# pirz/hyperspace-1

Measured on AMD Instinct MI355X. Metric: queries/sec + index-build GB/s, TPC-H SF100 filter+join at 1/2/4/8 MI355X, higher is better.
Workload: dtype fp64

## Files before the change

### csrc/kernels/scan_filter.hip

```cpp
#include "hs_vec.h"

#define SF_BLOCK 256
#define SF_ITEMS 8
#define SF_TILE (SF_BLOCK * SF_ITEMS)
#define SF_GRID 2048
#define FIN_BLOCK 256

struct ScanParams {
  ColDesc cols[HS_MAX_COLS];
  Pred preds[HS_MAX_PREDS];
  AggSpec aggs[HS_MAX_AGGS];
  int32_t npreds;
  int32_t naggs;
  int32_t group_col;
  int32_t num_groups;
  int64_t group_base;
};

#define RANGE_WAVES 4

__device__ __forceinline__ bool range_less(const ColDesc& c, int64_t r, uint64_t key, int mode) {
  if (!col_valid(c, r)) return true;
  if (mode == 2) return false;
  const uint64_t v = hs_sortable(c, r);
// ... 47 lines not shown
  range_one(key, bucket_off, buckets, i, has_lo, lo_key, lo_incl, has_hi, hi_key, hi_incl, rstart,
            rlen, rbucket);
}

__global__ __launch_bounds__(64 * RANGE_WAVES) void hs_probe_ranges_kernel(
    ColDesc key, const int64_t* __restrict__ bucket_off, const int32_t* __restrict__ pbucket,
    const uint64_t* __restrict__ pkey, int np, int64_t* __restrict__ rstart,
    int64_t* __restrict__ rlen, int32_t* __restrict__ rbucket) {
  const int i = blockIdx.x * RANGE_WAVES + (threadIdx.x >> 6);
  if (i >= np) return;
  range_one(key, bucket_off, pbucket, i, 1, pkey[i], 1, 1, pkey[i], 1, rstart, rlen, rbucket);
}

__global__ __launch_bounds__(64 * RANGE_WAVES) void hs_range_search_dev_kernel(
    ColDesc key, const int64_t* __restrict__ bucket_off, const int32_t* __restrict__ buckets,
    int nb, const int64_t* __restrict__ bp, int64_t* __restrict__ rstart,
    int64_t* __restrict__ rlen, int32_t* __restrict__ rbucket) {
  const int i = blockIdx.x * RANGE_WAVES + (threadIdx.x >> 6);
  if (i >= nb) return;
  range_one(key, bucket_off, buckets, i, (int)bp[0], (uint64_t)bp[1], (int)bp[2], (int)bp[3],
            (uint64_t)bp[4], (int)bp[5], rstart, rlen, rbucket);
}

__global__ __launch_bounds__(64) void hs_ranges_to_tiles_kernel(const int64_t* __restrict__ rlen,
                                                                int R, int tile_rows,
                                                                int64_t* __restrict__ tile_prefix,
                                                                const int64_t* __restrict__ rstart,
                                                                int64_t align) {
  const int lane = threadIdx.x & 63;
  int64_t carry = 0;
  for (int base = 0; base < R; base += 64) {
    const int i = base + lane;
    const int64_t len = i < R ? rlen[i] + (rstart != nullptr ? (rstart[i] & (align - 1)) : 0) : 0;
    const int64_t t = (len + tile_rows - 1) / tile_rows;
    int64_t x = t;
#pragma unroll
    for (int off = 1; off < 64; off <<= 1) {
      const int64_t y = __shfl_up(x, off, 64);
      if (lane >= off) x += y;
    }
    if (i < R) tile_prefix[i] = carry + x - t;
    carry += __shfl(x, 63, 64);
  }
  if (lane == 0) tile_prefix[R] = carry;
}

// ... 40 lines not shown
  int64_t t0, t1;
  block_tile_chunk(tile_prefix[R], t0, t1);
  if (t0 < t1) {
    TileWalker tw{tile_prefix, rstart, rlen, R, 0};
    tw.init(t0);
    for (int64_t t = t0; t < t1; ++t) {
      int64_t row0, rows;
      tw.at(t, row0, rows);
      int64_t r[SF_ITEMS];
      bool act[SF_ITEMS], pass[SF_ITEMS];
      tile_rows(row0, rows, r, act);
      veval_cnf(p.preds, 0, p.npreds, p.cols, HS_MAX_COLS, r, r, act, pass);
      int g[SF_ITEMS];
#pragma unroll
      for (int i = 0; i < SF_ITEMS; ++i) g[i] = 0;
      if (GROUPED)
        vgroup(p.cols, p.group_col, HS_MAX_COLS, p.group_base, p.num_groups, r, r, pass, g);
      vaccumulate<GROUPED, SF_ITEMS>(acc, p.aggs, A, p.cols, HS_MAX_COLS, r, r, pass, g, gl);
    }
  }
  acc_flush<GROUPED, SF_BLOCK>(acc, p.aggs, A, GA, gl, psum, pcnt, pmin, pmax);
}

__global__ __launch_bounds__(FIN_BLOCK) void hs_agg_final_kernel(
    const double* __restrict__ psum, const int64_t* __restrict__ pcnt,
    const double* __restrict__ pmin, const double* __restrict__ pmax, int nblk, int GA,
    double* __restrict__ osum, int64_t* __restrict__ ocnt, double* __restrict__ omin,
    double* __restrict__ omax) {
  __shared__ double rs[FIN_BLOCK / 64], rmn[FIN_BLOCK / 64], rmx[FIN_BLOCK / 64];
  __shared__ int64_t rc[FIN_BLOCK / 64];
  const int i = blockIdx.x;
  double s = 0.0, mn = __builtin_inf(), mx = -__builtin_inf();
  int64_t c = 0;
#pragma unroll 4
  for (int b = threadIdx.x; b < nblk; b += FIN_BLOCK) {
    const int64_t o = (int64_t)b * GA + i;
    s += psum[o];
    c += pcnt[o];
    mn = fmin(mn, pmin[o]);
    mx = fmax(mx, pmax[o]);
  }
  s = hs_wave_sum(s);
  c = hs_wave_sum(c);
  mn = hs_wave_min(mn);
  mx = hs_wave_max(mx);
  const int w = threadIdx.x >> 6;
  if ((threadIdx.x & 63) == 0) {
    rs[w] = s;
    rc[w] = c;
    rmn[w] = mn;
    rmx[w] = mx;
  }
  __syncthreads();
  if (threadIdx.x == 0) {
    double ts = 0.0, tmn = __builtin_inf(), tmx = -__builtin_inf();
    int64_t tc = 0;
    for (int k = 0; k < FIN_BLOCK / 64; ++k) {
      ts += rs[k];
      tc += rc[k];
      tmn = fmin(tmn, rmn[k]);
      tmx = fmax(tmx, rmx[k]);
    }
    osum[i] = ts;
    ocnt[i] = tc;
    omin[i] = tmn;
    omax[i] = tmx;
  }
}

__global__ __launch_bounds__(SF_BLOCK) void hs_scan_count_kernel(
    ScanParams p, const int64_t* __restrict__ rstart, const int64_t* __restrict__ rlen, int R,
    const int64_t* __restrict__ tile_prefix, int64_t* __restrict__ tile_counts) {
  __shared__ int64_t red[SF_BLOCK / 64];
  int64_t t0, t1;
  block_tile_chunk(tile_prefix[R], t0, t1);
  if (t0 >= t1) return;
  TileWalker tw{tile_prefix, rstart, rlen, R, 0};
  tw.init(t0);
  for (int64_t t = t0; t < t1; ++t) {
    int64_t row0, rows;
    tw.at(t, row0, rows);
    int64_t r[SF_ITEMS];
    bool act[SF_ITEMS], pass[SF_ITEMS];
    tile_rows(row0, rows, r, act);
    veval_cnf(p.preds, 0, p.npreds, p.cols, HS_MAX_COLS, r, r, act, pass);
    int64_t cnt = 0;
#pragma unroll
    for (int i = 0; i < SF_ITEMS; ++i) cnt += pass[i] ? 1 : 0;
    cnt = hs_wave_sum(cnt);
// ... 117 lines not shown
int hs_ranges_to_tiles(const int64_t* rlen, int R, int tile_rows, int64_t* tile_prefix,
                       void* stream) {
  hipLaunchKernelGGL(hs_ranges_to_tiles_kernel, dim3(1), dim3(64), 0, (hipStream_t)stream, rlen,
                     R, tile_rows, tile_prefix, (const int64_t*)nullptr, (int64_t)1);
  return (int)hipGetLastError();
}

int hs_ranges_to_tiles_aligned(const int64_t* rstart, const int64_t* rlen, int R, int tile_rows,
                               int64_t align, int64_t* tile_prefix, void* stream) {
  hipLaunchKernelGGL(hs_ranges_to_tiles_kernel, dim3(1), dim3(64), 0, (hipStream_t)stream, rlen,
                     R, tile_rows, tile_prefix, rstart, align);
  return (int)hipGetLastError();
}

int hs_agg_final(const double* psum, const int64_t* pcnt, const double* pmin, const double* pmax,
                 int nblk, int GA, double* osum, int64_t* ocnt, double* omin, double* omax,
                 void* stream) {
  if (GA <= 0) return 0;
  hipLaunchKernelGGL(hs_agg_final_kernel, dim3(GA), dim3(FIN_BLOCK), 0, (hipStream_t)stream, psum,
                     pcnt, pmin, pmax, nblk, GA, osum, ocnt, omin, omax);
  return (int)hipGetLastError();
}

int hs_scan_agg(const ScanParams* p, const int64_t* rstart, const int64_t* rlen, int R,
                const int64_t* tile_prefix, int grid, double* psum, int64_t* pcnt, double* pmin,
                double* pmax, double* osum, int64_t* ocnt, double* omin, double* omax,
                void* stream) {
  hipStream_t s = (hipStream_t)stream;
  const bool grouped = p->group_col >= 0;
  const int GA = grouped ? p->num_groups * p->naggs : p->naggs;
  if (GA <= 0) return 0;
  if (grouped) {
    const size_t lds = (size_t)GA * 32;
    if (lds > 120 * 1024) return -5;
    hipLaunchKernelGGL(hs_scan_agg_kernel<true>, dim3(grid), dim3(SF_BLOCK), lds, s, *p, rstart,
                       rlen, R, tile_prefix, psum, pcnt, pmin, pmax);
  } else {
    hipLaunchKernelGGL(hs_scan_agg_kernel<false>, dim3(grid), dim3(SF_BLOCK), 0, s, *p, rstart,
                       rlen, R, tile_prefix, psum, pcnt, pmin, pmax);
  }
  return hs_agg_final(psum, pcnt, pmin, pmax, grid, GA, osum, ocnt, omin, omax, stream);
}

int hs_scan_count(const ScanParams* p, const int64_t* rstart, const int64_t* rlen, int R,
                  const int64_t* tile_prefix, int grid, int64_t* tile_counts, void* stream) {
  hipLaunchKernelGGL(hs_scan_count_kernel, dim3(grid), dim3(SF_BLOCK), 0, (hipStream_t)stream, *p,
// ... 23 lines not shown
```

### csrc/runtime/hs_graph.cpp

```cpp
#include <hip/hip_runtime.h>

#include <algorithm>
#include <cstdint>
#include <cstring>
#include <string>
#include <vector>

namespace {

thread_local std::string g_err;

struct HsGraph {
  hipGraph_t graph = nullptr;
  hipGraphExec_t exec = nullptr;
  hipEvent_t join = nullptr;
  std::vector<hipGraphNode_t> nodes;
  std::vector<hipKernelNodeParams> params;
};

int fail(const char* what, hipError_t e) {
  g_err = std::string(what) + ": " + hipGetErrorString(e);
  return (int)e;
}

bool sort_by_depth(std::vector<hipGraphNode_t>& all) {
  const size_t n = all.size();
  std::vector<std::vector<size_t>> deps(n);
  for (size_t k = 0; k < n; ++k) {
    size_t nd = 0;
    if (hipGraphNodeGetDependencies(all[k], nullptr, &nd) != hipSuccess) return false;
    std::vector<hipGraphNode_t> d(nd);
    if (nd && hipGraphNodeGetDependencies(all[k], d.data(), &nd) != hipSuccess) return false;
    for (size_t j = 0; j < nd; ++j) {
      size_t at = 0;
      while (at < n && all[at] != d[j]) ++at;
      if (at == n) return false;
// ... 27 lines not shown
  all.swap(out);
  return true;
}

}

extern "C" {

const char* hs_graph_last_error() { return g_err.c_str(); }

int hs_graph_capture_begin(void* stream) {
  const hipError_t e = hipStreamBeginCapture((hipStream_t)stream, hipStreamCaptureModeThreadLocal);
  return e == hipSuccess ? 0 : fail("hipStreamBeginCapture", e);
}

void* hs_graph_capture_end(void* stream, void** funcs, int nfuncs) {
  hipGraph_t graph = nullptr;
  hipError_t e = hipStreamEndCapture((hipStream_t)stream, &graph);
  if (e != hipSuccess || graph == nullptr) {
    fail("hipStreamEndCapture", e);
    return nullptr;
  }
  auto* g = new HsGraph();
  g->graph = graph;
  size_t n = 0;
  e = hipGraphGetNodes(graph, nullptr, &n);
  std::vector<hipGraphNode_t> all(n);
  if (e == hipSuccess && n) e = hipGraphGetNodes(graph, all.data(), &n);
  if (e != hipSuccess) {
    fail("hipGraphGetNodes", e);
    hipGraphDestroy(graph);
    delete g;
    return nullptr;
  }
  all.resize(n);
  if (!sort_by_depth(all)) {
    g_err = "hs_graph_capture_end: could not order the captured nodes by dependency";
    hipGraphDestroy(graph);
    delete g;
    return nullptr;
  }
  std::vector<char> taken(n, 0);
  for (int i = 0; i < nfuncs; ++i) {
    bool found = false;
    for (size_t k = 0; k < n && !found; ++k) {
      if (taken[k]) continue;
      hipGraphNodeType t;
      if (hipGraphNodeGetType(all[k], &t) != hipSuccess || t != hipGraphNodeTypeKernel) continue;
      hipKernelNodeParams p;
      std::memset(&p, 0, sizeof(p));
      if (hipGraphKernelNodeGetParams(all[k], &p) != hipSuccess) continue;
      if (p.func != funcs[i]) continue;
      taken[k] = 1;
      g->nodes.push_back(all[k]);
      g->params.push_back(p);
      found = true;
    }
    if (!found) {
      g_err = "hs_graph_capture_end: kernel node of function " + std::to_string(i) + " not found";
      hipGraphDestroy(graph);
      delete g;
      return nullptr;
    }
  }
  e = hipGraphInstantiate(&g->exec, graph, nullptr, nullptr, 0);
  if (e != hipSuccess) {
    fail("hipGraphInstantiate", e);
    hipGraphDestroy(graph);
    delete g;
    return nullptr;
  }
  return g;
}

int hs_graph_set_args(void* handle, int i, void* args, size_t size) {
  auto* g = (HsGraph*)handle;
  if (i < 0 || (size_t)i >= g->nodes.size()) {
    g_err = "hs_graph_set_args: bad node index";
    return -1;
  }
  (void)size;
  hipKernelNodeParams p = g->params[i];
  void* kp[1] = {args};
  p.kernelParams = kp;
  p.extra = nullptr;
  const hipError_t e = hipGraphExecKernelNodeSetParams(g->exec, g->nodes[i], &p);
  return e == hipSuccess ? 0 : fail("hipGraphExecKernelNodeSetParams", e);
}

int hs_graph_launch(void* handle, void* stream) {
  auto* g = (HsGraph*)handle;
  const hipError_t e = hipGraphLaunch(g->exec, (hipStream_t)stream);
  return e == hipSuccess ? 0 : fail("hipGraphLaunch", e);
}

// ... 49 lines not shown
}

int hs_event_query(void* ev) {
  const hipError_t e = hipEventQuery((hipEvent_t)ev);
  if (e == hipSuccess) return 0;
  if (e == hipErrorNotReady) return 1;
  return -fail("hipEventQuery", e);
}

int hs_event_sync(void* ev) {
  const hipError_t e = hipEventSynchronize((hipEvent_t)ev);
  return e == hipSuccess ? 0 : fail("hipEventSynchronize", e);
}

void hs_event_destroy(void* ev) {
  if (ev != nullptr) hipEventDestroy((hipEvent_t)ev);
}

void hs_graph_destroy(void* handle) {
  auto* g = (HsGraph*)handle;
  if (g == nullptr) return;
  if (g->join) hipEventDestroy(g->join);
  if (g->exec) hipGraphExecDestroy(g->exec);
  if (g->graph) hipGraphDestroy(g->graph);
  delete g;
}

}
```

### hyperspace_amd/exec/graphs.py

```python
from __future__ import annotations

import ctypes as C
import struct
import threading
from collections import OrderedDict
from typing import Optional, Tuple

import numpy as np

from ..ops import _lib as NL
from . import jit

PARAM_HEAD = 64


class _Pinned:

    def __init__(self, nbytes: int):
        self.nbytes = nbytes
        self.ptr = jit.runtime().hs_host_alloc(nbytes)
        if not self.ptr:
            raise MemoryError(f"hipHostMalloc({nbytes}) failed")

    def view(self) -> np.ndarray:
        v = getattr(self, "_view", None)
        if v is None:
            v = self._view = np.ctypeslib.as_array((C.c_uint8 * self.nbytes).from_address(self.ptr))
        return v

    def __del__(self):
        if getattr(self, "ptr", None):
            jit.runtime().hs_host_free(self.ptr)
            self.ptr = None


class _Slot:

    def __init__(self, params_bytes: int, out_bytes: int):
        self.h_params = _Pinned(max(params_bytes, 8))
        self.h_out = _Pinned(out_bytes)
        self.graph = None
        self.event = jit.runtime().hs_event_create()
        if not self.event:
            raise RuntimeError(f"hs_event_create: {jit.runtime().hs_graph_last_error().decode()}")
        self.launched = False
        self.current = None

    def done(self) -> bool:
        rc = jit.runtime().hs_event_query(self.event)
        _rt_check(rc if rc < 0 else 0, "hs_event_query")
        return rc == 0

    def wait(self) -> None:
        _rt_check(jit.runtime().hs_event_sync(self.event), "hs_event_sync")

    def __del__(self):
        R = jit.runtime()
        if getattr(self, "graph", None):
            R.hs_graph_destroy(self.graph)
            self.graph = None
        if getattr(self, "event", None):
            R.hs_event_destroy(self.event)
            self.event = None


class _Launch:

    __slots__ = ("slot", "value")

    def __init__(self, slot: _Slot):
        self.slot = slot
        self.value = None


def _rt_check(rc: int, what: str) -> None:
    if rc != 0:
        raise RuntimeError(f"{what}: {jit.runtime().hs_graph_last_error().decode()}")


class _RingGraph:
    RING = 4

    def _init_ring(self, params_bytes: int) -> None:
        self.slots = [_Slot(params_bytes, self.out[0].hs_buf.numel()) for _ in range(self.RING)]
        self._next = 0
        self._warm = False
        self.replays = 0
        self.on_side = False
        self.side_stream = None

    @property
    def graph(self):
        return self.slots[0].graph

    def _capture(self, slot: _Slot, blocks, cur) -> None:
        slot.graph = self._capture_of(lambda st: self._enqueue(slot, st, blocks), self.kernels,
                                      cur)

    def _capture_of(self, enqueue, kernels, cur):
        import torch
        R = jit.runtime()
        side = torch.cuda.Stream()
        side.wait_stream(cur)
        _rt_check(R.hs_graph_capture_begin(side.cuda_stream), "hs_graph_capture_begin")
        try:
            enqueue(side.cuda_stream)
        finally:
            fns = [k.function() for k in kernels]
            arr = (C.c_void_p * len(fns))(*fns)
            h = R.hs_graph_capture_end(side.cuda_stream, arr, len(fns))
        if not h:
            raise RuntimeError(f"graph capture: {R.hs_graph_last_error().decode()}")
        cur.wait_stream(side)
        return h

    def _take_slot(self) -> _Slot:
        slot = self.slots[self._next]
        self._next = (self._next + 1) % len(self.slots)
        prev = slot.current
        if prev is not None and prev.value is None:
            prev.value = self._read(slot)
        elif slot.launched and not slot.done():
            slot.wait()
        return slot

    def busy(self) -> bool:
        slot = self.slots[self._next - 1]
        return slot.launched and not slot.done()

    def _launch_slot(self, fill, blocks, stream=None, after=None) -> _Launch:
        import torch
        slot = self._take_slot()
        fill(slot.h_params)
        R = jit.runtime()
        if slot.graph is not None:
            st = stream.cuda_stream if stream is not None else NL.raw_stream()
            ptrs = (C.c_void_p * len(blocks))(*[C.addressof(b) for b in blocks])
            _rt_check(R.hs_graph_replay(slot.graph, len(blocks), ptrs, st,
                                        after.cuda_stream if after is not None else None,
                                        slot.event), "hs_graph_replay")
            self.replays += 1
        else:
            cur = stream if stream is not None else torch.cuda.current_stream()
            st = cur.cuda_stream
            if after is not None:
                cur.wait_stream(after)
            if not self._warm:
                self._enqueue(slot, st, blocks)
                self._warm = True
            else:
                self._capture(slot, blocks, cur)
                _rt_check(R.hs_graph_launch(slot.graph, st), "hs_graph_launch")
                self.replays += 1
            _rt_check(R.hs_event_record(slot.event, st), "hs_event_record")
        slot.launched = True
        h = _Launch(slot)
        slot.current = h
        return h

    def result(self, h: _Launch):
        if h.value is None:
            h.value = self._read(h.slot)
        return h.value

    def _read(self, slot: _Slot):
        slot.wait()
        h = slot.h_out.view()
        n = 8 * self.GA
        return (h[0:n].view(np.float64).copy(), h[n:2 * n].view(np.int64).copy(),
                h[2 * n:3 * n].view(np.float64).copy(), h[3 * n:4 * n].view(np.float64).copy())

    def _final_and_d2h(self, slot: _Slot, stream: int, grid: int, parts=None) -> None:
        L = jit.runtime()
        K = NL.lib()
        p = self.parts if parts is None else parts
        o = self.out
        NL.check(K.hs_agg_final(NL.ptr(p[0]), NL.ptr(p[1]), NL.ptr(p[2]), NL.ptr(p[3]),
                                grid, self.GA, NL.ptr(o[0]), NL.ptr(o[1]), NL.ptr(o[2]),
                                NL.ptr(o[3]), stream), "hs_agg_final")
        NL.check(L.hs_memcpy_async(slot.h_out.ptr, o[0].hs_buf.data_ptr(), slot.h_out.nbytes, 2,
                                   stream), "result D2H")


def _cbuf(block) -> "C.Array":
    b = bytes(block)
    return C.create_string_buffer(b, len(b))


class ScanAggGraph(_RingGraph):
    def __init__(self, kernel: jit.Kernel, kd: NL.ColDesc, bucket_off, nb: int, grid: int,
                 GA: int, shmem: int, device, vec: int = 0):
        import torch
        from ..ops import kernels as K
        self.kernel = kernel
        self.kernels = (kernel,)
        self.kd = kd
        self.bucket_off = bucket_off
        self.nb, self.grid, self.GA, self.shmem = nb, grid, GA, shmem
        self.vec = vec
        self.tile = jit.BLOCK * (vec or jit.SCAN_ITEMS)
        self.d_params = torch.empty(PARAM_HEAD, dtype=torch.uint8, device=device)
        self.rstart = torch.empty(nb, dtype=torch.int64, device=device)
        self.rlen = torch.empty(nb, dtype=torch.int64, device=device)
        self.rbk = torch.empty(nb, dtype=torch.int32, device=device)
        self.tp = torch.empty(nb + 1, dtype=torch.int64, device=device)
        self.parts = jit._partials(grid, GA, device)
        self.out = K.agg_outputs(GA, device)
        self._init_ring(PARAM_HEAD)

    def _enqueue(self, slot: _Slot, stream: int, blocks) -> None:
        L = jit.runtime()
        K = NL.lib()
        NL.check(L.hs_memcpy_async(self.d_params.data_ptr(), slot.h_params.ptr,
                                   slot.h_params.nbytes, 1, stream), "param H2D")
        NL.check(K.hs_range_search_dev(C.byref(self.kd), NL.ptr(self.bucket_off), None, self.nb,
                                       self.d_params.data_ptr(), NL.ptr(self.rstart),
                                       NL.ptr(self.rlen), NL.ptr(self.rbk), stream),
                 "hs_range_search_dev")
        if self.vec:
            NL.check(K.hs_ranges_to_tiles_aligned(NL.ptr(self.rstart), NL.ptr(self.rlen), self.nb,
                                                  self.tile, self.vec, NL.ptr(self.tp), stream),
                     "hs_ranges_to_tiles_aligned")
        else:
            NL.check(K.hs_ranges_to_tiles(NL.ptr(self.rlen), self.nb, self.tile,
                                          NL.ptr(self.tp), stream), "hs_ranges_to_tiles")
        self.kernel.launch_packed(self.grid, blocks[0], stream, self.shmem)
        self._final_and_d2h(slot, stream, self.grid)

    def buffers(self) -> list:
        return [self.d_params, self.rstart, self.rlen, self.rbk, self.tp, self.bucket_off,
                *self.parts, self.out[0].hs_buf]

    def values_template(self) -> dict:
        return {"rstart": self.rstart.data_ptr(), "rlen": self.rlen.data_ptr(),
                "tile_prefix": self.tp.data_ptr(), "R": self.nb,
                "psum": self.parts[0].data_ptr(), "pcnt": self.parts[1].data_ptr(),
                "pmin": self.parts[2].data_ptr(), "pmax": self.parts[3].data_ptr()}

    def launch(self, bounds: Tuple[int, int, int, int, int, int], args_block, stream=None,
               after=None) -> _Launch:
        head = struct.pack("<6q", *bounds)

        def fill(hp):
            C.memmove(hp.ptr, head, 48)
        if not isinstance(args_block, C.Array):
            args_block = _cbuf(args_block)
        return self._launch_slot(fill, (args_block,), stream, after)

    def run(self, bounds: Tuple[int, int, int, int, int, int], args_block):
        return self.result(self.launch(bounds, args_block))


def _nofill(hp) -> None:
    pass


class TwoPhaseGraph(_RingGraph):

    def __init__(self, kt: jit.Kernel, ks: jit.Kernel, grid_t: int, grid_s: int, GA: int,
                 shmem: int, device):
        from ..ops import kernels as K
        self.kt, self.ks = kt, ks
        self.kernels = (kt, ks)
        self.grid_t, self.grid_s, self.GA, self.shmem = grid_t, grid_s, GA, shmem
        self.parts = jit._partials(grid_s, GA, device)
        self.parts_b = jit._partials(grid_s, GA, device)
        self.out = K.agg_outputs(GA, device)
        self._init_ring(0)
        self.pairs: dict = {}
        self._pair_warm = False
        self.pair_replays = 0

    def _enqueue(self, slot: _Slot, stream: int, blocks) -> None:
        self.kt.launch_packed(self.grid_t, blocks[0], stream, 0)
        self.ks.launch_packed(self.grid_s, blocks[1], stream, self.shmem)
        self._final_and_d2h(slot, stream, self.grid_s)

    def _enqueue_pair(self, ktp: jit.Kernel, sa: _Slot, sb: _Slot, stream: int, blocks,
                      ksp: Optional[jit.Kernel] = None) -> None:
        ktp.launch_packed(self.grid_t, blocks[0], stream, 0)
        if ksp is not None:
            ksp.launch_packed(self.grid_s, blocks[1], stream, self.shmem)
            self._final_and_d2h(sa, stream, self.grid_s)
            self._final_and_d2h(sb, stream, self.grid_s, self.parts_b)
            return
        for slot, blk in ((sa, blocks[1]), (sb, blocks[2])):
            self.ks.launch_packed(self.grid_s, blk, stream, self.shmem)
            self._final_and_d2h(slot, stream, self.grid_s)

    def launch_pair(self, ktp: jit.Kernel, block_tp, block_sa, block_sb, single,
                    ksp: Optional[jit.Kernel] = None) -> tuple:
        import torch
        ia = self._next
        sa, sb = self._take_slot(), self._take_slot()
        blocks = (block_tp, block_sa, block_sb) if ksp is None else (block_tp, block_sa)
        R = jit.runtime()
        h = self.pairs.get(ia)
        if h is not None:
            st = NL.raw_stream()
            ptrs = (C.c_void_p * len(blocks))(*[C.addressof(b) for b in blocks])
            _rt_check(R.hs_graph_replay(h, len(blocks), ptrs, st, None, sa.event),
                      "hs_graph_replay")
            self.pair_replays += 1
        else:
            cur = torch.cuda.current_stream()
            st = cur.cuda_stream
            if not self._pair_warm:
                self._enqueue_pair(ktp, sa, sb, st, blocks, ksp)
                self._pair_warm = True
            else:
                h = self.pairs[ia] = self._capture_of(
                    lambda s_: self._enqueue_pair(ktp, sa, sb, s_, blocks, ksp),
                    (ktp, self.ks, self.ks) if ksp is None else (ktp, ksp), cur)
                _rt_check(R.hs_graph_launch(h, st), "hs_graph_launch")
                self.pair_replays += 1
            _rt_check(R.hs_event_record(sa.event, st), "hs_event_record")
        _rt_check(R.hs_event_record(sb.event, st), "hs_event_record")
        out = []
        for slot in (sa, sb):
            slot.launched = True
            slot.current = _Launch(slot)
            out.append(slot.current)
        if self._warm and (sa.graph is None or sb.graph is None):
            self._capture(sa if sa.graph is None else sb, single, torch.cuda.current_stream())
        return tuple(out)

    def __del__(self):
        pairs = getattr(self, "pairs", None)
        while pairs:
            jit.runtime().hs_graph_destroy(pairs.popitem()[1])

    def buffers(self) -> list:
        return [*self.parts, *self.parts_b, self.out[0].hs_buf]

    def partial_ptrs(self, sfx: str = "", parts=None) -> dict:
        p = self.parts if parts is None else parts
        return {"psum" + sfx: p[0].data_ptr(), "pcnt" + sfx: p[1].data_ptr(),
                "pmin" + sfx: p[2].data_ptr(), "pmax" + sfx: p[3].data_ptr()}

    def launch(self, block_t, block_s) -> _Launch:
        return self._launch_slot(_nofill, (block_t, block_s))


class GraphPending:
    __slots__ = ("graph", "handle")

    def __init__(self, graph, handle):
        self.graph, self.handle = graph, handle

    def result(self):
        return self.graph.result(self.handle)

    def done(self) -> bool:
        h = self.handle
        return h.value is not None or h.slot.current is not h or h.slot.done()


class GraphCache:

    def __init__(self, capacity: int = 64):
        self.capacity = capacity
        self._lru: "OrderedDict[tuple, ScanAggGraph]" = OrderedDict()
        self._lock = threading.Lock()

# ... 34 lines not shown
```

### hyperspace_amd/exec/jit.py

```python
from __future__ import annotations

import ctypes as C
import os
import re
import struct
import threading
from typing import Dict, List, Optional, Tuple

from ..ops import _lib as NL

ARCH = os.environ.get("HS_OFFLOAD_ARCH", "gfx950")
_HERE = os.path.dirname(os.path.dirname(os.path.abspath(__file__)))
RUNTIME_PATH = os.path.join(_HERE, "_native", "libhs_runtime.so")
CACHE_DIR = os.environ.get("HS_JIT_CACHE", os.path.join(_HERE, "_native", "jitcache"))

BLOCK = 256
from . import kernel_config as _KC
_CFG = _KC.active()
SCAN_ITEMS, SCAN_GRID, SCAN_VEC = _CFG.scan_items, _CFG.scan_grid, _CFG.scan_vec
SCAN_COMPACT, SCAN_EAGER = _CFG.scan_compact, _CFG.scan_eager
JOIN_ITEMS, JOIN_BLOCK, JOIN_LDS_KEYS, JOIN_GRID = (_CFG.join_items, _CFG.join_block,
                                                    _CFG.join_lds_keys, _CFG.join_grid)
JOIN_EAGER, JOIN_STAGE_RIGHT, JOIN_PIPELINE = (_CFG.join_eager, _CFG.join_stage_right,
                                               _CFG.join_pipeline)
# ... 40 lines not shown
                L.hs_jit_launch.restype = C.c_int
                L.hs_jit_launch.argtypes = [C.c_void_p, C.c_uint, C.c_uint, C.c_uint, C.c_void_p,
                                            C.c_void_p, C.c_size_t]
                L.hs_jit_compile_to_cache.restype = C.c_int
                L.hs_jit_compile_to_cache.argtypes = [C.c_char_p] * 4
                L.hs_jit_last_error.restype = C.c_char_p
                L.hs_host_alloc.restype = C.c_void_p
                L.hs_host_alloc.argtypes = [C.c_size_t]
                L.hs_host_free.restype = None
                L.hs_host_free.argtypes = [C.c_void_p]
                L.hs_memcpy_async.restype = C.c_int
                L.hs_memcpy_async.argtypes = [C.c_void_p, C.c_void_p, C.c_size_t, C.c_int,
                                              C.c_void_p]
                L.hs_stream_sync.restype = C.c_int
                L.hs_stream_sync.argtypes = [C.c_void_p]
                L.hs_graph_capture_begin.restype = C.c_int
                L.hs_graph_capture_begin.argtypes = [C.c_void_p]
                L.hs_graph_capture_end.restype = C.c_void_p
                L.hs_graph_capture_end.argtypes = [C.c_void_p, C.POINTER(C.c_void_p), C.c_int]
                L.hs_graph_set_args.restype = C.c_int
                L.hs_graph_set_args.argtypes = [C.c_void_p, C.c_int, C.c_void_p, C.c_size_t]
                L.hs_graph_launch.restype = C.c_int
                L.hs_graph_launch.argtypes = [C.c_void_p, C.c_void_p]
                L.hs_graph_destroy.restype = None
                L.hs_graph_destroy.argtypes = [C.c_void_p]
                L.hs_graph_replay.restype = C.c_int
                L.hs_graph_replay.argtypes = [C.c_void_p, C.c_int, C.c_void_p, C.c_void_p,
                                              C.c_void_p, C.c_void_p]
                L.hs_event_create.restype = C.c_void_p
                L.hs_event_create.argtypes = []
                L.hs_event_record.restype = C.c_int
                L.hs_event_record.argtypes = [C.c_void_p, C.c_void_p]
                L.hs_event_query.restype = C.c_int
                L.hs_event_query.argtypes = [C.c_void_p]
                L.hs_event_sync.restype = C.c_int
                L.hs_event_sync.argtypes = [C.c_void_p]
                L.hs_event_destroy.restype = None
                L.hs_event_destroy.argtypes = [C.c_void_p]
                L.hs_graph_last_error.restype = C.c_char_p
                _rt = L
    return _rt


class Args:

    def __init__(self):
# ... 1804 lines not shown
```

### hyperspace_amd/ops/_lib.py

```python
from __future__ import annotations

import ctypes as C
import os

_HERE = os.path.dirname(os.path.dirname(os.path.abspath(__file__)))
LIB_PATH = os.path.join(_HERE, "_native", "libhs_kernels.so")

MAX_COLS = 16
MAX_PREDS = 16
MAX_AGGS = 8
MAX_TERMS = 3
HASH_MAX_COLS = 8
GATHER_MAX_COLS = 32

I8, I16, I32, I64, F32, F64, BOOL, U32, U64 = range(9)
STR = 100
STRDICT = 101
PK_INT_LIT, PK_FLT_LIT, PK_INT_COL, PK_FLT_COL, PK_IS_NULL, PK_NOT_NULL, PK_IN_SET, PK_BITMAP, \
    PK_TRUE = range(9)
OP_EQ, OP_NE, OP_LT, OP_LE, OP_GT, OP_GE = range(6)
AK_SUM, AK_COUNT, AK_MIN, AK_MAX, AK_COUNT_STAR = range(5)


class ColDesc(C.Structure):
# ... 65 lines not shown


XCH_MAX_COLS = 32
XCH_MAX_DEST = 64


class XchParams(C.Structure):
    _fields_ = [("src", C.c_void_p * XCH_MAX_COLS), ("elem_bytes", C.c_int32 * XCH_MAX_COLS),
                ("ncols", C.c_int32), ("world", C.c_int32)]


class XchCopy(C.Structure):
    _fields_ = [("src", C.c_void_p), ("dst", C.c_void_p), ("count", C.c_int64),
                ("elem_bytes", C.c_int32), ("pad", C.c_int32)]


WIN_MAX_KEYS = 8
WA_SUM_I64, WA_SUM_F64, WA_COUNT, WA_MIN_I64, WA_MAX_I64, WA_MIN_F64, WA_MAX_F64 = range(7)


class WinKeys(C.Structure):
    _fields_ = [("part", ColDesc * WIN_MAX_KEYS), ("order", ColDesc * WIN_MAX_KEYS),
                ("npart", C.c_int32), ("norder", C.c_int32)]


_lib = None


class NativeMissing(RuntimeError):
    pass


def _sig(fn, restype, *args):
    fn.restype = restype
    fn.argtypes = list(args)


def bind_hip_runtime() -> None:
    import torch


def lib():
    global _lib
    if _lib is not None:
        return _lib
    if not os.path.exists(LIB_PATH):
        raise NativeMissing(f"{LIB_PATH} not built; run `python -m hyperspace_amd._native.build`")
    bind_hip_runtime()
    L = C.CDLL(LIB_PATH)
    P, I, I64, U64 = C.c_void_p, C.c_int, C.c_int64, C.c_uint64
    for name, st in (("hs_hash_params_size", HashParams), ("hs_scan_params_size", ScanParams),
                     ("hs_join_params_size", JoinParams), ("hs_sort_key_spec_size", SortKeySpec),
                     ("hs_gather_params_size", GatherParams), ("hs_xch_params_size", XchParams),
                     ("hs_xch_copy_size", XchCopy), ("hs_merge_keys_size", MergeKeys),
                     ("hs_win_keys_size", WinKeys)):
        f = getattr(L, name)
        f.restype = C.c_int
        if f() != C.sizeof(st):
            raise RuntimeError(f"ABI mismatch for {st.__name__}: lib {f()} vs ctypes {C.sizeof(st)}")
    _sig(L.hs_murmur3_bucket, I, P, I64, P, P, P)
    _sig(L.hs_murmur3_hash, I, P, I64, P, P)
    _sig(L.hs_sort_workspace_bytes, I64, I64)
    _sig(L.hs_sort_columns, I, P, I, I64, P, I, P, I64, P)
    _sig(L.hs_merge_make_keys, I, P, I64, P, P)
    _sig(L.hs_merge_round, I, P, P, P, P, P, I, I64, P)
    _sig(L.hs_scan_tmp_elems, I64, I64)
    _sig(L.hs_exclusive_scan_i64, I, P, P, I64, P, I64, P)
    _sig(L.hs_exclusive_scan_u32, I, P, P, I64, P, I64, P)
    _sig(L.hs_gather, I, P, P, I64, P)
    _sig(L.hs_gather_packed, I, P, I, I, I64, P, P, I64, P)
    _sig(L.hs_bucket_offsets, I, P, I64, I, P, P)
    _sig(L.hs_scan_tile_rows, I)
    _sig(L.hs_scan_grid, I)
    _sig(L.hs_join_tile_rows, I)
    _sig(L.hs_range_search, I, P, P, P, I, I, U64, I, I, U64, I, P, P, P, P)
    _sig(L.hs_range_search_dev, I, P, P, P, I, P, P, P, P, P)
    _sig(L.hs_ranges_to_tiles, I, P, I, I, P, P)
    _sig(L.hs_ranges_to_tiles_aligned, I, P, P, I, I, I64, P, P)
    _sig(L.hs_scan_agg, I, P, P, P, I, P, I, P, P, P, P, P, P, P, P, P)
    _sig(L.hs_scan_count, I, P, P, P, I, P, I, P, P)
    _sig(L.hs_scan_select, I, P, P, P, I, P, P, I, P, P)
    _sig(L.hs_scan_bitmap, I, P, P, P, I, P, I, I, I64, I64, P, P)
    _sig(L.hs_join_agg, I, P, P, P, P, P, I, P, I64, P, I, P, P, P, P, P, P, P, P, P)
    _sig(L.hs_agg_final, I, P, P, P, P, I, I, P, P, P, P, P)
    _sig(L.hs_join_count, I, P, P, P, P, P, I, P, I64, P, I, P, P)
    _sig(L.hs_join_emit, I, P, I, P, P, I, P, P, P, P)
    _sig(L.hs_join_spans, I, P, P, P, P, P, I, P, I64, P, I, P)
    _sig(L.hs_join_spans_sampled, I, P, P, P, P, P, P, I, I64, P, I, P, I64, P, I, I, P)
    _sig(L.hs_join_sample_stride, I)
    _sig(L.hs_join_index, I, P, I, P, P, I, P, P)
    _sig(L.hs_pq_decode_values, I, P, P, I64, I64, I64, I, P, P)
    _sig(L.hs_pq_decode_levels, I, P, P, I64, P, P)
    _sig(L.hs_pq_pack, I, P, P, I, I64, I, P, P, P)
    _sig(L.hs_pq_dict_mark, I, P, P, I, I64, I, P, P)
    _sig(L.hs_pq_dict_remap, I, P, P, I, I64, I, P, P, P)
    _sig(L.hs_pq_warmup, I, P)
    _sig(L.hs_pq_decode_pages, I, P, P, P, I, P, P)
    _sig(L.hs_pq_page_struct_size, I)
    _sig(L.hs_pq_dict_codes, I, P, I64, I, P, I, P, P, P)
    _sig(L.hs_histogram, I, P, I64, I, P, P)
    _sig(L.hs_xch_tile_rows, I)
    _sig(L.hs_xch_pack, I, P, P, I64, P, P, P, P)
    _sig(L.hs_xch_unpack, I, P, I, I64, P)
    _sig(L.hs_probe_ranges, I, P, P, P, P, I, P, P, P, P)
    _sig(L.hs_compact_result_size, I)
    _sig(L.hs_compact_probe, I, P, P, I64, I, I, P, P, P)
    _sig(L.hs_compact_probe_ws_elems, I64)
# ... 87 lines not shown
```

Baseline: 4840.

## Fold aggregate finalisation with host write into kernel and clone captured graphs

Replaces the separate agg-final kernel plus D2H memcpy with a fold kernel that writes results straight into pinned host memory, using a system fence. Range-search parameters now travel by value in kernel arguments instead of through an H2D param copy. Graphs are captured once as a prototype and cloned for the other ring slots instead of being recaptured per slot. This removes memcpy graph nodes and repeated capture cost, at the price of system-scope device writes and graphs that share ownership.

```diff
diff --git a/csrc/kernels/scan_filter.hip b/csrc/kernels/scan_filter.hip
--- a/csrc/kernels/scan_filter.hip
+++ b/csrc/kernels/scan_filter.hip
@@ -93,6 +93,25 @@
             (uint64_t)bp[4], (int)bp[5], rstart, rlen, rbucket);
 }
 
+struct RangeValArgs {
+  ColDesc key;
+  const int64_t* bucket_off;
+  const int32_t* buckets;
+  int64_t* rstart;
+  int64_t* rlen;
+  int32_t* rbucket;
+  int64_t bp[6];
+  int32_t nb;
+  int32_t pad;
+};
+
+__global__ __launch_bounds__(64 * RANGE_WAVES) void hs_range_search_val_kernel(RangeValArgs a) {
+  const int i = blockIdx.x * RANGE_WAVES + (threadIdx.x >> 6);
+  if (i >= a.nb) return;
+  range_one(a.key, a.bucket_off, a.buckets, i, (int)a.bp[0], (uint64_t)a.bp[1], (int)a.bp[2],
+            (int)a.bp[3], (uint64_t)a.bp[4], (int)a.bp[5], a.rstart, a.rlen, a.rbucket);
+}
+
 __global__ __launch_bounds__(64) void hs_ranges_to_tiles_kernel(const int64_t* __restrict__ rlen,
                                                                 int R, int tile_rows,
                                                                 int64_t* __restrict__ tile_prefix,
@@ -179,14 +198,12 @@
   acc_flush<GROUPED, SF_BLOCK>(acc, p.aggs, A, GA, gl, psum, pcnt, pmin, pmax);
 }
 
-__global__ __launch_bounds__(FIN_BLOCK) void hs_agg_final_kernel(
+__device__ __forceinline__ bool agg_final_slot(
     const double* __restrict__ psum, const int64_t* __restrict__ pcnt,
-    const double* __restrict__ pmin, const double* __restrict__ pmax, int nblk, int GA,
-    double* __restrict__ osum, int64_t* __restrict__ ocnt, double* __restrict__ omin,
-    double* __restrict__ omax) {
+    const double* __restrict__ pmin, const double* __restrict__ pmax, int nblk, int GA, int i,
+    double& ts, int64_t& tc, double& tmn, double& tmx) {
   __shared__ double rs[FIN_BLOCK / 64], rmn[FIN_BLOCK / 64], rmx[FIN_BLOCK / 64];
   __shared__ int64_t rc[FIN_BLOCK / 64];
-  const int i = blockIdx.x;
   double s = 0.0, mn = __builtin_inf(), mx = -__builtin_inf();
   int64_t c = 0;
 #pragma unroll 4
@@ -209,19 +226,70 @@
     rmx[w] = mx;
   }
   __syncthreads();
-  if (threadIdx.x == 0) {
-    double ts = 0.0, tmn = __builtin_inf(), tmx = -__builtin_inf();
-    int64_t tc = 0;
-    for (int k = 0; k < FIN_BLOCK / 64; ++k) {
-      ts += rs[k];
-      tc += rc[k];
-      tmn = fmin(tmn, rmn[k]);
-      tmx = fmax(tmx, rmx[k]);
-    }
+  if (threadIdx.x != 0) return false;
+  ts = 0.0, tmn = __builtin_inf(), tmx = -__builtin_inf();
+  tc = 0;
+  for (int k = 0; k < FIN_BLOCK / 64; ++k) {
+    ts += rs[k];
+    tc += rc[k];
+    tmn = fmin(tmn, rmn[k]);
+    tmx = fmax(tmx, rmx[k]);
+  }
+  return true;
+}
+
+__global__ __launch_bounds__(FIN_BLOCK) void hs_agg_final_kernel(
+    const double* __restrict__ psum, const int64_t* __restrict__ pcnt,
+    const double* __restrict__ pmin, const double* __restrict__ pmax, int nblk, int GA,
+    double* __restrict__ osum, int64_t* __restrict__ ocnt, double* __restrict__ omin,
+    double* __restrict__ omax) {
+  const int i = blockIdx.x;
+  double ts, tmn, tmx;
+  int64_t tc;
+  if (agg_final_slot(psum, pcnt, pmin, pmax, nblk, GA, i, ts, tc, tmn, tmx)) {
     osum[i] = ts;
     ocnt[i] = tc;
     omin[i] = tmn;
     omax[i] = tmx;
+  }
+}
+
+struct AggFoldSet {
+  const double* psum;
+  const int64_t* pcnt;
+  const double* pmin;
+  const double* pmax;
+  unsigned char* dout;
+  unsigned char* hout;
+  int32_t nblk;
+  int32_t pad;
+};
+
+struct AggFoldArgs {
+  int32_t GA;
+  int32_t nsets;
+  AggFoldSet set[2];
+};
+
+__device__ __forceinline__ void agg_fold_store(unsigned char* __restrict__ out, int GA, int i,
+                                               double ts, int64_t tc, double tmn, double tmx) {
+  const size_t n = (size_t)8 * GA;
+  ((double*)out)[i] = ts;
+  ((int64_t*)(out + n))[i] = tc;
+  ((double*)(out + 2 * n))[i] = tmn;
+  ((double*)(out + 3 * n))[i] = tmx;
+}
+
+__global__ __launch_bounds__(FIN_BLOCK) void hs_agg_fold_kernel(AggFoldArgs a) {
+  const int k = blockIdx.x / a.GA, i = blockIdx.x - k * a.GA;
+  if (k >= a.nsets) return;
+  const AggFoldSet st = k == 0 ? a.set[0] : a.set[1];
+  double ts, tmn, tmx;
+  int64_t tc;
+  if (agg_final_slot(st.psum, st.pcnt, st.pmin, st.pmax, st.nblk, a.GA, i, ts, tc, tmn, tmx)) {
+    if (st.dout != nullptr) agg_fold_store(st.dout, a.GA, i, ts, tc, tmn, tmx);
+    agg_fold_store(st.hout, a.GA, i, ts, tc, tmn, tmx);
+    __threadfence_system();
   }
 }
 
@@ -385,6 +453,31 @@
   return (int)hipGetLastError();
 }
 
+int hs_agg_fold_args_size() { return (int)sizeof(AggFoldArgs); }
+
+void* hs_agg_fold_func() { return (void*)hs_agg_fold_kernel; }
+
+int hs_agg_fold(const AggFoldArgs* a, void* stream) {
+  if (a->GA <= 0) return 0;
+  if (a->nsets < 1 || a->nsets > 2) return -1;
+  for (int k = 0; k < a->nsets; ++k)
+    if (a->set[k].hout == nullptr || a->set[k].nblk < 0) return -1;
+  hipLaunchKernelGGL(hs_agg_fold_kernel, dim3(a->nsets * a->GA), dim3(FIN_BLOCK), 0,
+                     (hipStream_t)stream, *a);
+  return (int)hipGetLastError();
+}
+
+int hs_range_search_val_args_size() { return (int)sizeof(RangeValArgs); }
+
+void* hs_range_search_val_func() { return (void*)hs_range_search_val_kernel; }
+
+int hs_range_search_val(const RangeValArgs* a, void* stream) {
+  if (a->nb <= 0) return 0;
+  hipLaunchKernelGGL(hs_range_search_val_kernel, dim3((a->nb + RANGE_WAVES - 1) / RANGE_WAVES),
+                     dim3(64 * RANGE_WAVES), 0, (hipStream_t)stream, *a);
+  return (int)hipGetLastError();
+}
+
 int hs_scan_agg(const ScanParams* p, const int64_t* rstart, const int64_t* rlen, int R,
                 const int64_t* tile_prefix, int grid, double* psum, int64_t* pcnt, double* pmin,
                 double* pmax, double* osum, int64_t* ocnt, double* omin, double* omax,
diff --git a/csrc/runtime/hs_graph.cpp b/csrc/runtime/hs_graph.cpp
--- a/csrc/runtime/hs_graph.cpp
+++ b/csrc/runtime/hs_graph.cpp
@@ -3,6 +3,7 @@
 #include <algorithm>
 #include <cstdint>
 #include <cstring>
+#include <memory>
 #include <string>
 #include <vector>
 
@@ -11,7 +12,7 @@
 thread_local std::string g_err;
 
 struct HsGraph {
-  hipGraph_t graph = nullptr;
+  std::shared_ptr<ihipGraph> graph;
   hipGraphExec_t exec = nullptr;
   hipEvent_t join = nullptr;
   std::vector<hipGraphNode_t> nodes;
@@ -85,21 +86,19 @@
     return nullptr;
   }
   auto* g = new HsGraph();
-  g->graph = graph;
+  g->graph = std::shared_ptr<ihipGraph>(graph, [](hipGraph_t x) { hipGraphDestroy(x); });
   size_t n = 0;
   e = hipGraphGetNodes(graph, nullptr, &n);
   std::vector<hipGraphNode_t> all(n);
   if (e == hipSuccess && n) e = hipGraphGetNodes(graph, all.data(), &n);
   if (e != hipSuccess) {
     fail("hipGraphGetNodes", e);
-    hipGraphDestroy(graph);
     delete g;
     return nullptr;
   }
   all.resize(n);
   if (!sort_by_depth(all)) {
     g_err = "hs_graph_capture_end: could not order the captured nodes by dependency";
-    hipGraphDestroy(graph);
     delete g;
     return nullptr;
   }
@@ -121,7 +120,6 @@
     }
     if (!found) {
       g_err = "hs_graph_capture_end: kernel node of function " + std::to_string(i) + " not found";
-      hipGraphDestroy(graph);
       delete g;
       return nullptr;
     }
@@ -129,11 +127,51 @@
   e = hipGraphInstantiate(&g->exec, graph, nullptr, nullptr, 0);
   if (e != hipSuccess) {
     fail("hipGraphInstantiate", e);
-    hipGraphDestroy(graph);
     delete g;
     return nullptr;
   }
   return g;
+}
+
+void* hs_graph_clone(void* handle) {
+  auto* src = (HsGraph*)handle;
+  if (src == nullptr || !src->graph) {
+    g_err = "hs_graph_clone: no captured graph";
+    return nullptr;
+  }
+  auto* g = new HsGraph();
+  g->graph = src->graph;
+  g->nodes = src->nodes;
+  g->params = src->params;
+  const hipError_t e = hipGraphInstantiate(&g->exec, g->graph.get(), nullptr, nullptr, 0);
+  if (e != hipSuccess) {
+    fail("hipGraphInstantiate", e);
+    delete g;
+    return nullptr;
+  }
+  return g;
+}
+
+int hs_graph_node_counts(void* handle, int* kernels, int* memcpys, int* others) {
+  auto* g = (HsGraph*)handle;
+  size_t n = 0;
+  hipError_t e = hipGraphGetNodes(g->graph.get(), nullptr, &n);
+  std::vector<hipGraphNode_t> all(n);
+  if (e == hipSuccess && n) e = hipGraphGetNodes(g->graph.get(), all.data(), &n);
+  if (e != hipSuccess) return fail("hipGraphGetNodes", e);
+  int nk = 0, nm = 0, no = 0;
+  for (size_t k = 0; k < n; ++k) {
+    hipGraphNodeType t;
+    e = hipGraphNodeGetType(all[k], &t);
+    if (e != hipSuccess) return fail("hipGraphNodeGetType", e);
+    if (t == hipGraphNodeTypeKernel) ++nk;
+    else if (t == hipGraphNodeTypeMemcpy) ++nm;
+    else ++no;
+  }
+  *kernels = nk;
+  *memcpys = nm;
+  *others = no;
+  return 0;
 }
 
 int hs_graph_set_args(void* handle, int i, void* args, size_t size) {
@@ -229,7 +267,6 @@
   if (g == nullptr) return;
   if (g->join) hipEventDestroy(g->join);
   if (g->exec) hipGraphExecDestroy(g->exec);
-  if (g->graph) hipGraphDestroy(g->graph);
   delete g;
 }
 
diff --git a/hyperspace_amd/exec/graphs.py b/hyperspace_amd/exec/graphs.py
--- a/hyperspace_amd/exec/graphs.py
+++ b/hyperspace_amd/exec/graphs.py
@@ -1,8 +1,8 @@
 from __future__ import annotations
 
 import ctypes as C
-import struct
 import threading
+import time
 from collections import OrderedDict
 from typing import Optional, Tuple
 
@@ -11,7 +11,23 @@
 from ..ops import _lib as NL
 from . import jit
 
-PARAM_HEAD = 64
+STATS = {"captures": 0, "capture_s": 0.0, "clones": 0, "clone_s": 0.0}
+
+
+class _LibKernel:
+
+    def __init__(self, getter: str):
+        self.getter = getter
+        self._fn = None
+
+    def function(self):
+        if self._fn is None:
+            self._fn = getattr(NL.lib(), self.getter)()
+        return self._fn
+
+
+_FOLD = _LibKernel("hs_agg_fold_func")
+_RANGE = _LibKernel("hs_range_search_val_func")
 
 
 class _Pinned:
@@ -36,9 +52,9 @@
 
 class _Slot:
 
-    def __init__(self, params_bytes: int, out_bytes: int):
-        self.h_params = _Pinned(max(params_bytes, 8))
+    def __init__(self, out_bytes: int):
         self.h_out = _Pinned(out_bytes)
+        self.fold = None
         self.graph = None
         self.event = jit.runtime().hs_event_create()
         if not self.event:
@@ -78,13 +94,32 @@
         raise RuntimeError(f"{what}: {jit.runtime().hs_graph_last_error().decode()}")
 
 
+def _clone(h):
+    R = jit.runtime()
+    t0 = time.perf_counter()
+    c = R.hs_graph_clone(h)
+    STATS["clones"] += 1
+    STATS["clone_s"] += time.perf_counter() - t0
+    if not c:
+        raise RuntimeError(f"hs_graph_clone: {R.hs_graph_last_error().decode()}")
+    return c
+
+
+def node_counts(h) -> Tuple[int, int, int]:
+    k, m, o = C.c_int(0), C.c_int(0), C.c_int(0)
+    _rt_check(jit.runtime().hs_graph_node_counts(h, C.byref(k), C.byref(m), C.byref(o)),
+              "hs_graph_node_counts")
+    return k.value, m.value, o.value
+
+
 class _RingGraph:
     RING = 4
 
-    def _init_ring(self, params_bytes: int) -> None:
-        self.slots = [_Slot(params_bytes, self.out[0].hs_buf.numel()) for _ in range(self.RING)]
+    def _init_ring(self) -> None:
+        self.slots = [_Slot(self.out[0].hs_buf.numel()) for _ in range(self.RING)]
         self._next = 0
         self._warm = False
+        self._proto = None
         self.replays = 0
         self.on_side = False
         self.side_stream = None
@@ -93,13 +128,33 @@
     def graph(self):
         return self.slots[0].graph
 
+    def _fold_set(self, parts, nblk: int, slot: _Slot, dout: bool) -> NL.AggFoldSet:
+        return NL.AggFoldSet(parts[0].data_ptr(), parts[1].data_ptr(), parts[2].data_ptr(),
+                             parts[3].data_ptr(),
+                             self.out[0].hs_buf.data_ptr() if dout else None, slot.h_out.ptr,
+                             nblk, 0)
+
+    def _fold_args(self, slot: _Slot, nblk: int) -> NL.AggFoldArgs:
+        a = slot.fold
+        if a is None:
+            a = slot.fold = NL.AggFoldArgs(self.GA, 1)
+            a.set[0] = self._fold_set(self.parts, nblk, slot, True)
+        return a
+
+    def _fold(self, args: NL.AggFoldArgs, stream: int) -> None:
+        NL.check(NL.lib().hs_agg_fold(C.byref(args), stream), "hs_agg_fold")
+
     def _capture(self, slot: _Slot, blocks, cur) -> None:
-        slot.graph = self._capture_of(lambda st: self._enqueue(slot, st, blocks), self.kernels,
-                                      cur)
+        if self._proto is None:
+            self._proto = slot.graph = self._capture_of(
+                lambda st: self._enqueue(slot, st, blocks), self.kernels, cur)
+        else:
+            slot.graph = _clone(self._proto)
 
     def _capture_of(self, enqueue, kernels, cur):
         import torch
         R = jit.runtime()
+        t0 = time.perf_counter()
         side = torch.cuda.Stream()
         side.wait_stream(cur)
         _rt_check(R.hs_graph_capture_begin(side.cuda_stream), "hs_graph_capture_begin")
@@ -112,6 +167,8 @@
         if not h:
             raise RuntimeError(f"graph capture: {R.hs_graph_last_error().decode()}")
         cur.wait_stream(side)
+        STATS["captures"] += 1
+        STATS["capture_s"] += time.perf_counter() - t0
         return h
 
     def _take_slot(self) -> _Slot:
@@ -128,11 +185,17 @@
         slot = self.slots[self._next - 1]
         return slot.launched and not slot.done()
 
-    def _launch_slot(self, fill, blocks, stream=None, after=None) -> _Launch:
+    def _launch_slot(self, blocks_of, stream=None, after=None) -> _Launch:
         import torch
         slot = self._take_slot()
-        fill(slot.h_params)
+        blocks = blocks_of(slot)
         R = jit.runtime()
+        if slot.graph is None and self._warm:
+            self._capture(slot, blocks,
+                          stream if stream is not None else torch.cuda.current_stream())
+            for other in self.slots:
+                if other.graph is None:
+                    other.graph = _clone(self._proto)
         if slot.graph is not None:
             st = stream.cuda_stream if stream is not None else NL.raw_stream()
             ptrs = (C.c_void_p * len(blocks))(*[C.addressof(b) for b in blocks])
@@ -145,13 +208,8 @@
             st = cur.cuda_stream
             if after is not None:
                 cur.wait_stream(after)
-            if not self._warm:
-                self._enqueue(slot, st, blocks)
-                self._warm = True
-            else:
-                self._capture(slot, blocks, cur)
-                _rt_check(R.hs_graph_launch(slot.graph, st), "hs_graph_launch")
-                self.replays += 1
+            self._enqueue(slot, st, blocks)
+            self._warm = True
             _rt_check(R.hs_event_record(slot.event, st), "hs_event_record")
         slot.launched = True
         h = _Launch(slot)
@@ -170,17 +228,6 @@
         return (h[0:n].view(np.float64).copy(), h[n:2 * n].view(np.int64).copy(),
                 h[2 * n:3 * n].view(np.float64).copy(), h[3 * n:4 * n].view(np.float64).copy())
 
-    def _final_and_d2h(self, slot: _Slot, stream: int, grid: int, parts=None) -> None:
-        L = jit.runtime()
-        K = NL.lib()
-        p = self.parts if parts is None else parts
-        o = self.out
-        NL.check(K.hs_agg_final(NL.ptr(p[0]), NL.ptr(p[1]), NL.ptr(p[2]), NL.ptr(p[3]),
-                                grid, self.GA, NL.ptr(o[0]), NL.ptr(o[1]), NL.ptr(o[2]),
-                                NL.ptr(o[3]), stream), "hs_agg_final")
-        NL.check(L.hs_memcpy_async(slot.h_out.ptr, o[0].hs_buf.data_ptr(), slot.h_out.nbytes, 2,
-                                   stream), "result D2H")
-
 
 def _cbuf(block) -> "C.Array":
     b = bytes(block)
@@ -193,30 +240,27 @@
         import torch
         from ..ops import kernels as K
         self.kernel = kernel
-        self.kernels = (kernel,)
+        self.kernels = (_RANGE, kernel, _FOLD)
         self.kd = kd
         self.bucket_off = bucket_off
         self.nb, self.grid, self.GA, self.shmem = nb, grid, GA, shmem
         self.vec = vec
         self.tile = jit.BLOCK * (vec or jit.SCAN_ITEMS)
-        self.d_params = torch.empty(PARAM_HEAD, dtype=torch.uint8, device=device)
         self.rstart = torch.empty(nb, dtype=torch.int64, device=device)
         self.rlen = torch.empty(nb, dtype=torch.int64, device=device)
         self.rbk = torch.empty(nb, dtype=torch.int32, device=device)
         self.tp = torch.empty(nb + 1, dtype=torch.int64, device=device)
         self.parts = jit._partials(grid, GA, device)
         self.out = K.agg_outputs(GA, device)
-        self._init_ring(PARAM_HEAD)
+        self._init_ring()
+        for slot in self.slots:
+            slot.range = NL.RangeValArgs(kd, bucket_off.data_ptr(), None, self.rstart.data_ptr(),
+                                         self.rlen.data_ptr(), self.rbk.data_ptr(),
+                                         (C.c_int64 * 6)(), nb, 0)
 
     def _enqueue(self, slot: _Slot, stream: int, blocks) -> None:
-        L = jit.runtime()
         K = NL.lib()
-        NL.check(L.hs_memcpy_async(self.d_params.data_ptr(), slot.h_params.ptr,
-                                   slot.h_params.nbytes, 1, stream), "param H2D")
-        NL.check(K.hs_range_search_dev(C.byref(self.kd), NL.ptr(self.bucket_off), None, self.nb,
-                                       self.d_params.data_ptr(), NL.ptr(self.rstart),
-                                       NL.ptr(self.rlen), NL.ptr(self.rbk), stream),
-                 "hs_range_search_dev")
+        NL.check(K.hs_range_search_val(C.byref(blocks[0]), stream), "hs_range_search_val")
         if self.vec:
             NL.check(K.hs_ranges_to_tiles_aligned(NL.ptr(self.rstart), NL.ptr(self.rlen), self.nb,
                                                   self.tile, self.vec, NL.ptr(self.tp), stream),
@@ -224,11 +268,11 @@
         else:
             NL.check(K.hs_ranges_to_tiles(NL.ptr(self.rlen), self.nb, self.tile,
                                           NL.ptr(self.tp), stream), "hs_ranges_to_tiles")
-        self.kernel.launch_packed(self.grid, blocks[0], stream, self.shmem)
-        self._final_and_d2h(slot, stream, self.grid)
+        self.kernel.launch_packed(self.grid, blocks[1], stream, self.shmem)
+        self._fold(blocks[2], stream)
 
     def buffers(self) -> list:
-        return [self.d_params, self.rstart, self.rlen, self.rbk, self.tp, self.bucket_off,
+        return [self.rstart, self.rlen, self.rbk, self.tp, self.bucket_off,
                 *self.parts, self.out[0].hs_buf]
 
     def values_template(self) -> dict:
@@ -239,20 +283,16 @@
 
     def launch(self, bounds: Tuple[int, int, int, int, int, int], args_block, stream=None,
                after=None) -> _Launch:
-        head = struct.pack("<6q", *bounds)
-
-        def fill(hp):
-            C.memmove(hp.ptr, head, 48)
         if not isinstance(args_block, C.Array):
             args_block = _cbuf(args_block)
-        return self._launch_slot(fill, (args_block,), stream, after)
+
+        def blocks_of(slot):
+            slot.range.bp[:] = bounds
+            return slot.range, args_block, self._fold_args(slot, self.grid)
+        return self._launch_slot(blocks_of, stream, after)
 
     def run(self, bounds: Tuple[int, int, int, int, int, int], args_block):
         return self.result(self.launch(bounds, args_block))
-
-
-def _nofill(hp) -> None:
-    pass
 
 
 class TwoPhaseGraph(_RingGraph):
@@ -261,59 +301,76 @@
                  shmem: int, device):
         from ..ops import kernels as K
         self.kt, self.ks = kt, ks
-        self.kernels = (kt, ks)
+        self.kernels = (kt, ks, _FOLD)
         self.grid_t, self.grid_s, self.GA, self.shmem = grid_t, grid_s, GA, shmem
         self.parts = jit._partials(grid_s, GA, device)
         self.parts_b = jit._partials(grid_s, GA, device)
         self.out = K.agg_outputs(GA, device)
-        self._init_ring(0)
+        self._init_ring()
         self.pairs: dict = {}
+        self._pair_proto = None
+        self._pair_folds: dict = {}
         self._pair_warm = False
         self.pair_replays = 0
 
     def _enqueue(self, slot: _Slot, stream: int, blocks) -> None:
         self.kt.launch_packed(self.grid_t, blocks[0], stream, 0)
         self.ks.launch_packed(self.grid_s, blocks[1], stream, self.shmem)
-        self._final_and_d2h(slot, stream, self.grid_s)
-
-    def _enqueue_pair(self, ktp: jit.Kernel, sa: _Slot, sb: _Slot, stream: int, blocks,
+        self._fold(blocks[2], stream)
+
+    def _pair_fold(self, ia: int, sa: _Slot, sb: _Slot) -> NL.AggFoldArgs:
+        a = self._pair_folds.get(ia)
+        if a is None:
+            a = self._pair_folds[ia] = NL.AggFoldArgs(self.GA, 2)
+            a.set[0] = self._fold_set(self.parts, self.grid_s, sa, False)
+            a.set[1] = self._fold_set(self.parts_b, self.grid_s, sb, True)
+        return a
+
+    def _enqueue_pair(self, ktp: jit.Kernel, stream: int, blocks,
                       ksp: Optional[jit.Kernel] = None) -> None:
         ktp.launch_packed(self.grid_t, blocks[0], stream, 0)
         if ksp is not None:
             ksp.launch_packed(self.grid_s, blocks[1], stream, self.shmem)
-            self._final_and_d2h(sa, stream, self.grid_s)
-            self._final_and_d2h(sb, stream, self.grid_s, self.parts_b)
+            self._fold(blocks[2], stream)
             return
-        for slot, blk in ((sa, blocks[1]), (sb, blocks[2])):
+        for blk, fold in ((blocks[1], blocks[2]), (blocks[3], blocks[4])):
             self.ks.launch_packed(self.grid_s, blk, stream, self.shmem)
-            self._final_and_d2h(slot, stream, self.grid_s)
+            self._fold(fold, stream)
 
     def launch_pair(self, ktp: jit.Kernel, block_tp, block_sa, block_sb, single,
                     ksp: Optional[jit.Kernel] = None) -> tuple:
         import torch
         ia = self._next
         sa, sb = self._take_slot(), self._take_slot()
-        blocks = (block_tp, block_sa, block_sb) if ksp is None else (block_tp, block_sa)
+        if ksp is not None:
+            blocks = (block_tp, block_sa, self._pair_fold(ia, sa, sb))
+            kernels = (ktp, ksp, _FOLD)
+        else:
+            blocks = (block_tp, block_sa, self._fold_args(sa, self.grid_s),
+                      block_sb, self._fold_args(sb, self.grid_s))
+            kernels = (ktp, self.ks, _FOLD, self.ks, _FOLD)
         R = jit.runtime()
         h = self.pairs.get(ia)
+        if h is None and self._pair_warm:
+            if self._pair_proto is None:
+                self._pair_proto = h = self._capture_of(
+                    lambda s_: self._enqueue_pair(ktp, s_, blocks, ksp), kernels,
+                    torch.cuda.current_stream())
+                for i in range(len(self.slots)):
+                    if i != ia:
+                        self.pairs[i] = _clone(h)
+            else:
+                h = _clone(self._pair_proto)
+            self.pairs[ia] = h
+        st = NL.raw_stream()
         if h is not None:
-            st = NL.raw_stream()
             ptrs = (C.c_void_p * len(blocks))(*[C.addressof(b) for b in blocks])
             _rt_check(R.hs_graph_replay(h, len(blocks), ptrs, st, None, sa.event),
                       "hs_graph_replay")
             self.pair_replays += 1
         else:
-            cur = torch.cuda.current_stream()
-            st = cur.cuda_stream
-            if not self._pair_warm:
-                self._enqueue_pair(ktp, sa, sb, st, blocks, ksp)
-                self._pair_warm = True
-            else:
-                h = self.pairs[ia] = self._capture_of(
-                    lambda s_: self._enqueue_pair(ktp, sa, sb, s_, blocks, ksp),
-                    (ktp, self.ks, self.ks) if ksp is None else (ktp, ksp), cur)
-                _rt_check(R.hs_graph_launch(h, st), "hs_graph_launch")
-                self.pair_replays += 1
+            self._enqueue_pair(ktp, st, blocks, ksp)
+            self._pair_warm = True
             _rt_check(R.hs_event_record(sa.event, st), "hs_event_record")
         _rt_check(R.hs_event_record(sb.event, st), "hs_event_record")
         out = []
@@ -322,7 +379,9 @@
             slot.current = _Launch(slot)
             out.append(slot.current)
         if self._warm and (sa.graph is None or sb.graph is None):
-            self._capture(sa if sa.graph is None else sb, single, torch.cuda.current_stream())
+            slot = sa if sa.graph is None else sb
+            self._capture(slot, (*single, self._fold_args(slot, self.grid_s)),
+                          torch.cuda.current_stream())
         return tuple(out)
 
     def __del__(self):
@@ -339,7 +398,8 @@
                 "pmin" + sfx: p[2].data_ptr(), "pmax" + sfx: p[3].data_ptr()}
 
     def launch(self, block_t, block_s) -> _Launch:
-        return self._launch_slot(_nofill, (block_t, block_s))
+        return self._launch_slot(
+            lambda slot: (block_t, block_s, self._fold_args(slot, self.grid_s)))
 
 
 class GraphPending:
diff --git a/hyperspace_amd/exec/jit.py b/hyperspace_amd/exec/jit.py
--- a/hyperspace_amd/exec/jit.py
+++ b/hyperspace_amd/exec/jit.py
@@ -86,6 +86,11 @@
                 L.hs_graph_set_args.argtypes = [C.c_void_p, C.c_int, C.c_void_p, C.c_size_t]
                 L.hs_graph_launch.restype = C.c_int
                 L.hs_graph_launch.argtypes = [C.c_void_p, C.c_void_p]
+                L.hs_graph_clone.restype = C.c_void_p
+                L.hs_graph_clone.argtypes = [C.c_void_p]
+                L.hs_graph_node_counts.restype = C.c_int
+                L.hs_graph_node_counts.argtypes = [C.c_void_p, C.POINTER(C.c_int),
+                                                   C.POINTER(C.c_int), C.POINTER(C.c_int)]
                 L.hs_graph_destroy.restype = None
                 L.hs_graph_destroy.argtypes = [C.c_void_p]
                 L.hs_graph_replay.restype = C.c_int
diff --git a/hyperspace_amd/ops/_lib.py b/hyperspace_amd/ops/_lib.py
--- a/hyperspace_amd/ops/_lib.py
+++ b/hyperspace_amd/ops/_lib.py
@@ -111,6 +111,22 @@
 class WinKeys(C.Structure):
     _fields_ = [("part", ColDesc * WIN_MAX_KEYS), ("order", ColDesc * WIN_MAX_KEYS),
                 ("npart", C.c_int32), ("norder", C.c_int32)]
+
+
+class AggFoldSet(C.Structure):
+    _fields_ = [("psum", C.c_void_p), ("pcnt", C.c_void_p), ("pmin", C.c_void_p),
+                ("pmax", C.c_void_p), ("dout", C.c_void_p), ("hout", C.c_void_p),
+                ("nblk", C.c_int32), ("pad", C.c_int32)]
+
+
+class AggFoldArgs(C.Structure):
+    _fields_ = [("GA", C.c_int32), ("nsets", C.c_int32), ("set", AggFoldSet * 2)]
+
+
+class RangeValArgs(C.Structure):
+    _fields_ = [("key", ColDesc), ("bucket_off", C.c_void_p), ("buckets", C.c_void_p),
+                ("rstart", C.c_void_p), ("rlen", C.c_void_p), ("rbucket", C.c_void_p),
+                ("bp", C.c_int64 * 6), ("nb", C.c_int32), ("pad", C.c_int32)]
 
 
 _lib = None
@@ -142,7 +158,8 @@
                      ("hs_join_params_size", JoinParams), ("hs_sort_key_spec_size", SortKeySpec),
                      ("hs_gather_params_size", GatherParams), ("hs_xch_params_size", XchParams),
                      ("hs_xch_copy_size", XchCopy), ("hs_merge_keys_size", MergeKeys),
-                     ("hs_win_keys_size", WinKeys)):
+                     ("hs_win_keys_size", WinKeys), ("hs_agg_fold_args_size", AggFoldArgs),
+                     ("hs_range_search_val_args_size", RangeValArgs)):
         f = getattr(L, name)
         f.restype = C.c_int
         if f() != C.sizeof(st):
@@ -172,6 +189,10 @@
     _sig(L.hs_scan_bitmap, I, P, P, P, I, P, I, I, I64, I64, P, P)
     _sig(L.hs_join_agg, I, P, P, P, P, P, I, P, I64, P, I, P, P, P, P, P, P, P, P, P)
     _sig(L.hs_agg_final, I, P, P, P, P, I, I, P, P, P, P, P)
+    _sig(L.hs_agg_fold, I, P, P)
+    _sig(L.hs_agg_fold_func, P)
+    _sig(L.hs_range_search_val, I, P, P)
+    _sig(L.hs_range_search_val_func, P)
     _sig(L.hs_join_count, I, P, P, P, P, P, I, P, I64, P, I, P, P)
     _sig(L.hs_join_emit, I, P, I, P, P, I, P, P, P, P)
     _sig(L.hs_join_spans, I, P, P, P, P, P, I, P, I64, P, I, P)
```

Result: faster. 4990 (median of 6 runs) (+3.1%).
